# google/supersonic

Hardware: AMD Instinct MI355X
Metric: rows/sec filter->project->aggregate, 100M x 8 INT64/DOUBLE (higher is better)
Workload: dtype int64/f64; 1 GPU; Q-FPA-wide: SUM(a+b),COUNT(*),SUM(c),MIN(d),MAX(d0),SUM(d1),SUM(d2*d3) WHERE a>499 over a device-resident 100000000-row x 8-col block per GPU; rows_per_gpu=100000000, parallelism=single GPU, tile_rows=512, grid=768, lds_bytes=35568, specialized_stages=1

## Files before the change

include/ssgpu.h:

```cpp
#ifndef SSGPU_H_
#define SSGPU_H_

#include <stddef.h>
#include <stdint.h>

#ifdef __cplusplus
extern "C" {
#endif

#define SSGPU_ABI_VERSION 10

enum {
  SSGPU_INT32 = 1, SSGPU_INT64 = 2, SSGPU_UINT64 = 3, SSGPU_DATETIME = 4,
  SSGPU_DOUBLE = 5, SSGPU_BOOL = 6, SSGPU_UINT32 = 8, SSGPU_FLOAT = 9,
  SSGPU_DATE = 10, SSGPU_STRING = 0, SSGPU_BINARY = 7
};
enum { SSGPU_NOT_NULLABLE = 0, SSGPU_NULLABLE = 1 };
enum {
  SSGPU_SUM = 0, SSGPU_MIN = 1, SSGPU_MAX = 2, SSGPU_COUNT = 3,
  SSGPU_CONCAT = 4, SSGPU_FIRST = 5, SSGPU_LAST = 6,
  SSGPU_SUM_RESIDUAL = 100
};
enum { SSGPU_ASCENDING = 0, SSGPU_DESCENDING = 1 };
enum {
// ... 223 lines not shown
int64_t ssgpu_plan_memory_in_use(const ssgpu_plan* plan);

typedef struct ssgpu_stage_info {
  int32_t kind;
  int32_t group_shape;
  int32_t part_n;
  int32_t part_seg_growth;
  int32_t group_wgs_per_cu;
  int32_t reruns;
  int32_t sort_passes;
  int32_t sort_mode;
  int32_t specialized;
  int32_t plain_scatter;
  int32_t hot_keys;
  int32_t dense_slots;
  int32_t reserved[4];
} ssgpu_stage_info;
int32_t ssgpu_plan_stage_count(const ssgpu_plan* plan);
int ssgpu_plan_stage_info(const ssgpu_plan* plan, int32_t stage, ssgpu_stage_info* out);

int ssgpu_expr_bind(ssgpu_ctx* ctx, const ssgpu_attr* schema, int32_t n_attrs, const ssgpu_expr* exprs, int32_t n_exprs,
                    const int32_t* expr_args, int32_t n_expr_args, int32_t root, int64_t max_row_count, ssgpu_plan** out);
int64_t ssgpu_expr_row_capacity(const ssgpu_plan* bound);
int ssgpu_expr_evaluate(ssgpu_plan* bound, const ssgpu_column* cols, int32_t n_cols, int64_t rows, ssgpu_result** out);
int ssgpu_expr_evaluate_skip(ssgpu_plan* bound, const ssgpu_column* cols, int32_t n_cols, int64_t rows, uint8_t* const* skip, int32_t n_skip,
                             ssgpu_result** out);

int ssgpu_plan_set_option(ssgpu_plan* plan, const char* key, int64_t value);
int ssgpu_plan_run_best_effort(ssgpu_plan* plan, const ssgpu_column* cols, int32_t n_cols, int64_t rows, int64_t start_row,
                               int64_t* next_row, ssgpu_result** out);
int ssgpu_plan_run(ssgpu_plan* plan, const ssgpu_column* cols, int32_t n_cols,
// ... 74 lines not shown
```

supersonic_amd/_lib.py:

```python
import ctypes as C
import os

_HERE = os.path.dirname(os.path.abspath(__file__))
LIB_PATH = os.environ.get("SSGPU_LIB") or os.path.join(_HERE, "lib", "libssgpu.so")

INT32, INT64, UINT64, DATETIME, DOUBLE, BOOL, UINT32, FLOAT, DATE, STRING, BINARY = 1, 2, 3, 4, 5, 6, 8, 9, 10, 0, 7
NOT_NULLABLE, NULLABLE = 0, 1
SUM, MIN, MAX, COUNT, CONCAT, FIRST, LAST = 0, 1, 2, 3, 4, 5, 6
SUM_RESIDUAL = 100
ASCENDING, DESCENDING = 0, 1

OK = 0
ERROR_UNKNOWN = 100
ERROR_GENERAL_IO_ERROR = 101
ERROR_MEMORY_EXCEEDED = 102
ERROR_NOT_IMPLEMENTED = 103
ERROR_EVALUATION_ERROR = 104
ERROR_TOO_MANY_ROWS = 302
ERROR_ATTRIBUTE_COUNT_MISMATCH = 401
ERROR_ATTRIBUTE_TYPE_MISMATCH = 402
ERROR_ATTRIBUTE_MISSING = 403
ERROR_ATTRIBUTE_EXISTS = 404
ERROR_INVALID_ARGUMENT_TYPE = 405
ERROR_INVALID_ARGUMENT_VALUE = 407
# ... 37 lines not shown

class Op(C.Structure):
    _fields_ = [("kind", C.c_int32), ("child", C.c_int32), ("expr", C.c_int32), ("proj_first", C.c_int32),
                ("proj_n", C.c_int32), ("agg_first", C.c_int32), ("agg_n", C.c_int32), ("sort_first", C.c_int32),
                ("sort_n", C.c_int32), ("child2", C.c_int32), ("option0", C.c_int64),
                ("proj2_first", C.c_int32), ("proj2_n", C.c_int32), ("proj3_first", C.c_int32), ("proj3_n", C.c_int32)]


class MemoryStats(C.Structure):
    _fields_ = [(n, C.c_int64) for n in ("device_bytes", "pinned_bytes", "live_plans", "live_blocks", "events",
                                          "rtc_modules", "rtc_code_bytes", "rtc_compilations", "rtc_disk_hits")]


class StageInfo(C.Structure):
    _fields_ = [(n, C.c_int32) for n in ("kind", "group_shape", "part_n", "part_seg_growth", "group_wgs_per_cu", "reruns",
                                          "sort_passes", "sort_mode", "specialized", "plain_scatter", "hot_keys", "dense_slots")] + [("reserved", C.c_int32 * 4)]


class PlanDesc(C.Structure):
    _fields_ = [("input_schema", C.POINTER(Attr)), ("n_attrs", C.c_int32),
                ("ops", C.POINTER(Op)), ("n_ops", C.c_int32),
                ("exprs", C.POINTER(Expr)), ("n_exprs", C.c_int32),
                ("expr_args", C.POINTER(C.c_int32)), ("n_expr_args", C.c_int32),
                ("projs", C.POINTER(Proj)), ("n_projs", C.c_int32),
                ("aggs", C.POINTER(Agg)), ("n_aggs", C.c_int32),
                ("sortkeys", C.POINTER(SortKey)), ("n_sortkeys", C.c_int32),
                ("aux_schema", C.POINTER(Attr)), ("n_aux_attrs", C.c_int32)]


class Column(C.Structure):
    _fields_ = [("data", C.c_void_p), ("is_null", C.c_void_p)]
# ... 158 lines not shown
```

supersonic_amd/csrc/engine.h:

```cpp
#ifndef SSGPU_ENGINE_H_
#define SSGPU_ENGINE_H_

#include <stdint.h>
#include <map>
#include <memory>
#include <string>
#include <vector>

#include "../../include/ssgpu.h"
#include "vm.h"
#include "launch.h"

extern "C" int ssgpu_dict_create_sorted(const char* heap, const uint64_t* offsets, int64_t n, ssgpu_dict** out);

namespace ssgpu {

struct Status {
  int code = SSGPU_OK;
  std::string msg;
  bool ok() const { return code == SSGPU_OK; }
  static Status OK() { return Status(); }
  static Status Error(int c, const std::string& m) { Status s; s.code = c; s.msg = m; return s; }
};
#define SS_RETURN_IF_ERROR(expr) do { ::ssgpu::Status _s = (expr); if (!_s.ok()) return _s; } while (0)
// ... 69 lines not shown
  uint16_t op = 0;
  bool a_imm = false, b_imm = false;
  uint8_t imm_width = 8;
  bool dst_is_reg = true;
  int dst = -1;
  int a = -1, b = -1, c = -1, d = -1, e = -1;
  uint64_t imm = 0;
};
struct StagedInput { int col; bool is_null_mask; int reg; };

struct Program {
  std::vector<LInstr> code;
  std::vector<LReg> regs;
  std::vector<StagedInput> staged;
  std::vector<JoinGather> gathers;
  bool uses_math = false;
  uint32_t bytes_per_row = 0;
  uint32_t in_bytes_per_row = 0;
  int n_slots = 0;
  int n_outputs = 0;
  bool empty() const { return code.empty(); }
};

struct Stage {
  StageKind kind = STAGE_MATERIALIZE;
  Schema in_schema;
  Schema out_schema;
  Program main;
  Program count_pass;
  bool has_filter = false;
// ... 73 lines not shown
```

supersonic_amd/csrc/launch.h:

```cpp
#ifndef SSGPU_LAUNCH_H_
#define SSGPU_LAUNCH_H_

#ifndef __HIPCC_RTC__
#include <hip/hip_runtime_api.h>
#include <stdint.h>
#endif
#include "vm.h"

enum SlotKind {
  SLOT_SUM_INT = 0, SLOT_SUM_DD = 1, SLOT_MIN_U64 = 2, SLOT_MAX_U64 = 3, SLOT_MIN_F64 = 4,
  SLOT_MAX_F64 = 5, SLOT_FIRST = 6, SLOT_LAST = 7, SLOT_COUNT = 8
};
enum EmitKind {
  EMIT_U64 = 0, EMIT_I64KEY = 1, EMIT_U32 = 2, EMIT_I32KEY = 3, EMIT_F64 = 4, EMIT_F32 = 5,
  EMIT_DD_F64 = 6, EMIT_DD_F32 = 7, EMIT_U8 = 8,
  EMIT_DDRES_F64 = 9,
  EMIT_CNT_U64 = 20, EMIT_CNT_U32 = 21,
  EMIT_FKEY_F64 = 100, EMIT_FKEY_F32 = 101
};
#define SSGPU_STATE_ARRAYS 8

struct EmitDesc { void* data; uint8_t* is_null; int slot; int out_kind; };

struct GroupKeyOut { void* data; uint8_t* is_null; uint32_t shift, bits, nullbit, width; };
// ... 145 lines not shown
hipError_t ssgpu_launch_join_build(const JoinBuildParams& P, hipStream_t stream);
hipError_t ssgpu_launch_fill_u32(unsigned int* p, unsigned int v, size_t n, hipStream_t stream);
struct GroupInitParams {
  unsigned long long* keys; unsigned long long n_keys;
  unsigned long long* acc; const unsigned long long* pattern; unsigned int ng; unsigned long long n_acc;
  unsigned int* cnt; unsigned long long n_cnt;
  unsigned int* z[4]; unsigned long long nz[4];
  unsigned int n_rep, pad; unsigned long long rep_stride;
};
hipError_t ssgpu_launch_group_init(const GroupInitParams& P, hipStream_t stream);

hipError_t ssgpu_launch_pipeline(const VmParams& P, int K, int grid, hipStream_t stream);
#ifndef __HIPCC_RTC__
#include <string>
void* ssgpu_rtc_specialize(int device, const VmInstr* prog, int n_instr, int K, bool math, const uint32_t* staged_width, const uint32_t* staged_lds_off,
                           int n_staged, uint32_t static_lds, std::string* why);
hipError_t ssgpu_launch_pipeline_rtc(void* handle, const VmParams& P, int grid, bool static_lds, hipStream_t stream);
void* ssgpu_rtc_specialize_part_agg(int device, const unsigned long long* desc, int n_aggs, unsigned int rec_words, unsigned int n_gaggs, bool any_cnt,
                                    unsigned int lds_bytes, std::string* why, const PlainScatterParams* source = nullptr,
                                    bool dense = false,
                                    bool prefetch = false);
hipError_t ssgpu_launch_group_resident_rtc(void* handle, const PartAggParams& A, const PlainScatterParams& S, int grid, hipStream_t stream);
hipError_t ssgpu_launch_part_agg_rtc(void* handle, const PartAggParams& P, hipStream_t stream);
void* ssgpu_rtc_specialize_pscat(int device, const PlainScatterParams& S, const PscatGeom& g, std::string* why);
hipError_t ssgpu_launch_part_scatter_plain_rtc(void* handle, const PlainScatterParams& P, const PscatGeom& g, int grid, hipStream_t stream);
void* ssgpu_rtc_function(void* handle);
void ssgpu_rtc_release(void* handle);
void ssgpu_rtc_cached_only(bool on);
void ssgpu_rtc_mode(int mode);
int ssgpu_rtc_current_mode();
bool ssgpu_rtc_pending();
// ... 107 lines not shown
```

supersonic_amd/csrc/lower.cpp:

```cpp
#include "engine.h"

#include <algorithm>
#include <functional>
#include <sstream>
#include <string.h>

namespace ssgpu {

enum {
  OP_ADD = 0, OP_MULTIPLY = 4, OP_SUBTRACT = 8, OP_DIVIDE_QUIET = 13, OP_DIVIDE_NULLING = 14,
  OP_DIVIDE_SIGNALING = 15, OP_CPP_DIVIDE_NULLING = 18, OP_CPP_DIVIDE_SIGNALING = 19,
  OP_MODULUS_NULLING = 26, OP_MODULUS_SIGNALING = 27, OP_NEGATE = 36,
  OP_IS_ODD = 140, OP_IS_EVEN = 144, OP_IS_FINITE = 148, OP_IS_INF = 152, OP_IS_NAN = 156, OP_IS_NORMAL = 160,
  OP_ROUND_WITH_MULTIPLIER = 364, OP_EXP = 320, OP_LN_QUIET = 325, OP_LN_NULLING = 326, OP_LOG10_QUIET = 329, OP_LOG10_NULLING = 330, OP_POW_QUIET = 353,
  OP_POW_NULLING = 354, OP_POW_SIGNALING = 355, OP_LOG2_QUIET = 357, OP_LOG2_NULLING = 358, OP_SIN = 800, OP_COS = 804, OP_TAN = 808,
  OP_ASIN = 812, OP_ACOS = 816, OP_ATAN = 820, OP_ATAN2 = 824, OP_SINH = 828, OP_COSH = 832, OP_TANH = 836, OP_ASINH = 840,
  OP_ACOSH = 844, OP_ATANH = 848,
  OP_ROUND = 300, OP_TRUNC = 304, OP_CEIL_TO_INT = 308, OP_FLOOR_TO_INT = 312, OP_SQRT_QUIET = 333, OP_SQRT_NULLING = 334,
  OP_SQRT_SIGNALING = 335, OP_CEIL = 342, OP_FLOOR = 346, OP_ABS = 360, OP_AND = 40, OP_OR = 44,
  OP_AND_NOT = 48, OP_NOT = 52, OP_XOR = 56, OP_BITWISE_AND = 60, OP_BITWISE_OR = 64,
  OP_BITWISE_NOT = 68, OP_BITWISE_XOR = 72, OP_SHIFT_LEFT = 76, OP_SHIFT_RIGHT = 80,
  OP_BITWISE_ANDNOT = 84, OP_EQUAL = 100, OP_NOT_EQUAL = 104, OP_LESS = 116, OP_LESS_OR_EQUAL = 120,
  OP_IF = 204, OP_IF_NULL = 220, OP_IS_NULL = 224, OP_CAST_QUIET = 265
};
// ... 689 lines not shown
    if (fused_agg) {
      v.b = off(i.b);
      if (i.b_imm) v.d = pool;
    }
    v.imm = i.imm;
    if (i.op == VM_AND3 || i.op == VM_OR3) v.imm = (uint64_t)off(i.d) | ((uint64_t)off(i.e) << 32);
    out->push_back(v);
  }
  VmInstr nop; memset(&nop, 0, sizeof(nop)); nop.op = VM_NOP;
  nop.dst = nop.a = nop.b = nop.c = nop.d = VM_NONE;
  out->push_back(nop);
}

std::string disassemble(const Program& p) {
  std::ostringstream s;
  s << "  staged:";
  for (auto& st : p.staged) s << " r" << st.reg << "<-col" << st.col << (st.is_null_mask ? ".null" : "") << "(w" << p.regs[st.reg].width << ")";
  s << "\n  lds bytes/row: " << p.bytes_per_row << ", slots: " << p.n_slots << ", outputs: " << p.n_outputs << "\n";
  auto R = [&](int r) { return r < 0 ? std::string("-") : "r" + std::to_string(r) + "@" + std::to_string(p.regs[r].row_off); };
  for (size_t pc = 0; pc < p.code.size(); ++pc) {
    const LInstr& i = p.code[pc];
    s << "  " << pc << ": " << vm_op_name(i.op) << " dst=" << (i.dst_is_reg ? R(i.dst) : "#" + std::to_string(i.dst))
      << " a=" << (i.a_imm ? "imm" : R(i.a)) << " b=" << (i.b_imm ? "imm" : R(i.b)) << " c=" << R(i.c) << " d=" << R(i.d);
    if (i.e >= 0) s << " e=" << R(i.e);
    if (i.a_imm || i.b_imm || i.imm) s << " imm=0x" << std::hex << i.imm << std::dec;
    s << "\n";
  }
  return s.str();
}

// ... 210 lines not shown
    Val pv;
    SS_RETURN_IF_ERROR(em.value(pipe.filters[f], &pv));
    if (!pv.imm && pv.null < 0 && em.sel_by_depth.back() < 0) {
      em.sel_by_depth.push_back(pv.reg);
      continue;
    }
    int r = em.new_reg(1);
    LInstr& i = em.emit(VM_SEL_FROM_PRED);
    i.dst = r;
    if (pv.imm) { i.a_imm = true; i.imm = pv.bits; i.imm_width = 1; } else i.a = pv.reg;
    i.b = pv.null;
    i.c = em.sel_by_depth.back();
    em.sel_by_depth.push_back(r);
  }
  return Status::OK();
}

static int64_t staged_bytes(const Program& p) {
  int64_t b = 0;
  for (auto& s : p.staged) b += p.regs[s.reg].width;
  return b;
}

static bool has_sequential(const std::vector<AggPlan>& plans) { for (auto& ap : plans) if (ap.sequential) return true; return false; }
static Status take_sequential(std::vector<AggPlan>* plans, const Pipe& pipe, size_t first_out, std::vector<Stage::SeqSum>* out) {
  for (size_t j = 0; j < plans->size(); ++j) {
    AggPlan& ap = (*plans)[j];
    if (!ap.sequential) continue;
    const BExprP& src = pipe.cols[ap.input_pos].expr;
    if (src->kind != BExpr::INPUT) return Status::Error(SSGPU_ERROR_NOT_IMPLEMENTED, "SUM of a floating value into an integer output needs a stored input column");
// ... 88 lines not shown
        if (ap.distinct) { int nf; SS_RETURN_IF_ERROR(notfirst_for(ap, &nf)); nullreg = em.or_null(v.null, nf); }
        int order_reg = -1;
        if (ap.order_pos >= 0 && (ap.aggregation == SSGPU_FIRST || ap.aggregation == SSGPU_LAST)) {
          Val ov; SS_RETURN_IF_ERROR(em.value(pipe.cols[ap.order_pos].expr, &ov));
          order_reg = em.materialize(ov);
        }
        LInstr& i = em.emit(s.op); i.dst_is_reg = false; i.dst = (int)j; i.a = vr; i.b = nullreg; i.c = sel; i.d = order_reg;
      }
      ao.slot_kind = s.slot_kind; ao.emit_kind = s.emit_kind;
    }
    st->aggs.push_back(ao);
    Attr a; a.name = ap.out_name; a.dtype = ap.out_type; a.nullable = ap.result_nullable;
    st->out_schema.push_back(a);
  }
  st->main.n_slots = (int)plans.size();
  allocate_registers(&st->main);
  st->algorithmic_bytes_per_row = staged_bytes(st->main);
  st->has_filter = !pipe.filters.empty();
  return Status::OK();
}

static Status finish_scalar_agg(const PlanDesc& d, const ssgpu_op& op, const Pipe& pipe, Stage* st) {
  std::vector<AggPlan> plans;
  SS_RETURN_IF_ERROR(bind_aggregations(d, op.agg_first, op.agg_n, schema_of(pipe.cols), &plans));
  return finish_scalar_agg_bound(plans, pipe, st);
}

struct AggPlan;
static Status build_partition_programs(const struct Pipe& pipe, const std::vector<int>& kpos, const std::vector<AggPlan>& plans, Stage* st);

// ... 406 lines not shown
    if (st->has_filter) { i.b = rank; i.c = sel; }
  };
  for (size_t c = 0; c < pipe.cols.size(); ++c) {
    const BExprP& e = pipe.cols[c].expr;
    Val v; SS_RETURN_IF_ERROR(em.value(e, &v));
    store(v, v.width);
    if (e->nullable) {
      Val nv; nv.width = 1;
      if (v.null >= 0) nv.reg = v.null; else { nv.imm = true; nv.bits = 0; }
      store(nv, 1);
    }
    st->output_bytes_per_row += v.width + (e->nullable ? 1 : 0);
  }
  if (out_index > VM_MAX_OUTPUTS) return Status::Error(SSGPU_ERROR_NOT_IMPLEMENTED, "too many output columns for one pipeline");
  st->main.n_outputs = out_index;
  allocate_registers(&st->main);
  st->algorithmic_bytes_per_row = staged_bytes(st->main);
  return Status::OK();
}

static Pipe prune_to_used(const Pipe& pipe, std::vector<int>* kpos, std::vector<AggPlan>* plans) {
  std::vector<int> used;
  auto slot_of = [&](int pos) { for (size_t i = 0; i < used.size(); ++i) if (used[i] == pos) return (int)i; used.push_back(pos); return (int)used.size() - 1; };
  if (kpos) for (auto& k : *kpos) k = slot_of(k);
  for (auto& ap : *plans) if (ap.input_pos >= 0) ap.input_pos = slot_of(ap.input_pos);
  Pipe pruned = pipe; pruned.cols.clear();
  for (size_t i = 0; i < used.size(); ++i) { VCol c = pipe.cols[used[i]]; c.name = "c" + std::to_string(i); pruned.cols.push_back(c); }
  return pruned;
}
static int add_row_id_column(Pipe* pruned) {
// ... 633 lines not shown
```

supersonic_amd/csrc/pipeline_kernels.hip:

```cpp
#ifndef __HIPCC_RTC__
#include <hip/hip_runtime.h>
#include <stdint.h>
#endif
#include "vm.h"
#include "launch.h"
#ifdef SSGPU_RTC_NINSTR
#include "rtc_prog.h"
#endif

typedef unsigned long long u64;
typedef long long i64;
typedef unsigned int u32;
typedef int i32;
typedef unsigned char u8;

#ifdef SSGPU_PC_PROFILE
#define PC_PROF(...) __VA_ARGS__
#else
#define PC_PROF(...)
#endif
struct LdsBase {
  __device__ __forceinline__ char* operator+(u32 off) const {
    return (char*)(__attribute__((address_space(3))) char*)off;
  }
// ... 151 lines not shown
  return 0xFFFFFFFFu;
}

typedef u32 u32x4 __attribute__((ext_vector_type(4)));
typedef u32 u32x2 __attribute__((ext_vector_type(2)));

#if defined(SSGPU_RTC_NINSTR) && !defined(SSGPU_RTC_DYNAMIC_STAGING)
#define STAGED_WIDTH(P, s) kRtcStagedWidth[s]
#define STAGED_LDS_OFF(P, s) kRtcStagedOff[s]
#define STAGED_COUNT(P) SSGPU_RTC_NSTAGED
#else
#define STAGED_WIDTH(P, s) (P).staged[s].width
#define STAGED_LDS_OFF(P, s) (P).staged[s].lds_off
#define STAGED_COUNT(P) (P).n_staged
#endif
template <int K>
__device__ __forceinline__ void load_unit(const VmParams& P, int u, i64 tile_base, int t, u32x4& v) {
  const int s = u / K, k = u % K;
  const char* const src0 = reinterpret_cast<const char*>(P.staged[s].src);
  const u32 w = STAGED_WIDTH(P, s);
  if (src0 == nullptr) return;
  const u32 p = (u32)(k * VM_COMPUTE_THREADS + t);
  if (w == 8) {
    v = __builtin_nontemporal_load(reinterpret_cast<const u32x4*>(src0 + (tile_base << 3) + (size_t)(p * 16u)));
  } else if (w == 4) {
    const u32x2 x = __builtin_nontemporal_load(reinterpret_cast<const u32x2*>(src0 + (tile_base << 2) + (size_t)(p * 8u)));
    v[0] = x[0]; v[1] = x[1];
  } else if ((reinterpret_cast<uintptr_t>(src0) & 1) == 0) {
    v[0] = (u32)__builtin_nontemporal_load(reinterpret_cast<const unsigned short*>(src0 + tile_base + (size_t)(p * 2u)));
  } else {
// ... 2 lines not shown
  }
}

template <int K>
__device__ __forceinline__ void commit_unit(const VmParams& P, int u, u32x4 v, int t) {
  const int s = u / K, k = u % K;
  const u32 w = STAGED_WIDTH(P, s);
  const u32 p = (u32)(k * VM_COMPUTE_THREADS + t);
  char* const dst = smem + STAGED_LDS_OFF(P, s);
  if (w == 8) *reinterpret_cast<u32x4*>(dst + p * 16u) = v;
  else if (w == 4) { u32x2 x = {v[0], v[1]}; *reinterpret_cast<u32x2*>(dst + p * 8u) = x; }
  else *reinterpret_cast<unsigned short*>(dst + p * 2u) = (unsigned short)v[0];
}

template <int K>
__device__ __forceinline__ void stage_units_direct(const VmParams& P, int u_begin, int u_end, i64 tile_base, u32 tile_valid, int t) {
  for (int u = u_begin; u < u_end; ++u) {
    const int s = u / K, k = u % K;
    const char* const src0 = reinterpret_cast<const char*>(P.staged[s].src);
    const u32 w = STAGED_WIDTH(P, s);
    const u32 p = (u32)(k * VM_COMPUTE_THREADS + t), r0 = 2u * p;
    char* const dst = smem + STAGED_LDS_OFF(P, s);
    const bool v0 = src0 != nullptr && r0 < tile_valid, v1 = src0 != nullptr && r0 + 1u < tile_valid;
    if (w == 8) {
      const u64* src = reinterpret_cast<const u64*>(src0) + tile_base + r0;
      u64 a = v0 ? src[0] : 0ull, b = v1 ? src[1] : 0ull;
      reinterpret_cast<u64*>(dst)[r0] = a; reinterpret_cast<u64*>(dst)[r0 + 1u] = b;
    } else if (w == 4) {
      const u32* src = reinterpret_cast<const u32*>(src0) + tile_base + r0;
      u32 a = v0 ? src[0] : 0u, b = v1 ? src[1] : 0u;
      reinterpret_cast<u32*>(dst)[r0] = a; reinterpret_cast<u32*>(dst)[r0 + 1u] = b;
    } else {
      const u8* src = reinterpret_cast<const u8*>(src0) + tile_base + r0;
      u8 a = v0 ? src[0] : (u8)0, b = v1 ? src[1] : (u8)0;
      reinterpret_cast<u8*>(dst)[r0] = a; reinterpret_cast<u8*>(dst)[r0 + 1u] = b;
    }
  }
}
// ... 337 lines not shown
  PC_PROF(if (P.debug_pc) for (int i = t; i <= P.n_instr; i += VM_COMPUTE_THREADS) reinterpret_cast<u64*>(smem + P.debug_pc_lds_off)[i] = 0ull;)
  __syncthreads();

  u32x4 pf[VM_PF_UNITS];
#pragma unroll
  for (int u = 0; u < VM_PF_UNITS; ++u) pf[u] = u32x4{0u, 0u, 0u, 0u};
  const int n_pf = n_units < VM_PF_UNITS ? n_units : VM_PF_UNITS;
  {
    const i64 tb = (i64)vm_first_tile * tile_rows;
    if (n_my_tiles > 0 && tb + tile_rows <= vm_n_rows) {
#pragma unroll
      for (int u = 0; u < VM_PF_UNITS; ++u)
        if (u < n_pf) load_unit<K>(P, u, tb, t, pf[u]);
    }
  }

  u64 dbg_wait = 0;
  const u64 dbg_t0 = P.debug ? __builtin_amdgcn_s_memtime() : 0;
  const ProgPtr prog = prog0;
  for (int it = 0; it < n_my_tiles; ++it) {
    const int tile = vm_first_tile + it * (int)gridDim.x;
    const i64 tile_base = (i64)tile * tile_rows;
    const u32 tile_valid = (u32)((vm_n_rows - tile_base) < (i64)tile_rows ? (vm_n_rows - tile_base) : (i64)tile_rows);
    const u64 tw0 = (P.debug || P.debug_pc) ? __builtin_amdgcn_s_memtime() : 0;
    __builtin_amdgcn_s_setprio(VM_STAGE_PRIO);
    if (tile_valid == (u32)tile_rows) {
      int tc = t;
      asm volatile("" : "+v"(tc));
#pragma unroll
      for (int u = 0; u < VM_PF_UNITS; ++u)
        if (u < n_pf) commit_unit<K>(P, u, pf[u], tc);
      if (P.debug) dbg_wait += __builtin_amdgcn_s_memtime() - tw0;
      if (n_units > VM_PF_UNITS) stage_units_direct<K>(P, VM_PF_UNITS, n_units, tile_base, tile_valid, t);
    } else {
      stage_units_direct<K>(P, 0, n_units, tile_base, tile_valid, t);
    }
    {
      const i64 tb = tile_base + (i64)gridDim.x * tile_rows;
      if (it + 1 < n_my_tiles && tb + tile_rows <= vm_n_rows) {
        int tl = t;
        asm volatile("" : "+v"(tl));
#pragma unroll
        for (int u = 0; u < VM_PF_UNITS; ++u)
          if (u < n_pf) load_unit<K>(P, u, tb, tl, pf[u]);
      }
    }

    __builtin_amdgcn_s_setprio(0);
#ifdef SSGPU_RTC_NINSTR
#define VM_PC_LOOP _Pragma("unroll") for (int pc = 0; pc < SSGPU_RTC_NINSTR; ++pc)
#define VM_FETCH_NEXT(pc) u32x8{kRtcProg[pc][0], kRtcProg[pc][1], kRtcProg[pc][2], kRtcProg[pc][3], kRtcProg[pc][4], kRtcProg[pc][5], kRtcProg[pc][6], kRtcProg[pc][7]}
    (void)prog;
    u32x8 raw_next = VM_FETCH_NEXT(0);
#else
#define VM_PC_LOOP for (int pc = 0; pc < P.n_instr; ++pc)
#define VM_FETCH_NEXT(pc) prog[pc]
    u32x8 raw_next = prog[0];
#endif
    PC_PROF(u64 dbg_pc_last = 0;
    if (P.debug_pc) { dbg_pc_last = __builtin_amdgcn_s_memtime(); if (t == 0) reinterpret_cast<u64*>(smem + P.debug_pc_lds_off)[P.n_instr] += dbg_pc_last - tw0; })
#ifdef SSGPU_RTC_NINSTR
#include "rtc_steps.h"
#else
    VM_PC_LOOP {
#include "vm_body.inc"
    }
#endif
    PC_PROF(if (P.debug_pc && P.n_instr > 0 && t == 0) reinterpret_cast<u64*>(smem + P.debug_pc_lds_off)[P.n_instr - 1] += __builtin_amdgcn_s_memtime() - dbg_pc_last;)
  }

  if (vm_nan_seen && P.error_flag) atomicOr(P.error_flag, SSGPU_FLAG_NAN_IN_MINMAX);
  if (P.part_n && P.tile_counts) {
    __syncthreads();
    const u32* h = reinterpret_cast<const u32*>(smem + P.part_lds_off);
    for (u32 i = (u32)t; i < P.part_n; i += VM_COMPUTE_THREADS) P.tile_counts[(u64)i * gridDim.x + blockIdx.x] = h[i] < P.part_seg_cap ? h[i] : P.part_seg_cap;
  }
  if (P.group.local_capacity) {
    const VmGroupTable& G = P.group;
    __syncthreads();
    const u32 ng = G.n_gaggs;
    u32 occupied = 0;
    for (u32 e = (u32)t; e < G.local_capacity; e += VM_COMPUTE_THREADS) {
      const u64 key = reinterpret_cast<const u64*>(smem + G.local_keys_off)[e];
// ... 1283 lines not shown
```

supersonic_amd/csrc/rtc.cpp:

```cpp
#include <dirent.h>
#include <dlfcn.h>
#include <fcntl.h>
#include <errno.h>
#include <sys/stat.h>
#include <sys/types.h>
#include <unistd.h>
#include <hip/hip_runtime_api.h>
#include <stdint.h>
#include <stdio.h>
#include <stdlib.h>
#include <string.h>

#include <algorithm>
#include <atomic>
#include <condition_variable>
#include <deque>
#include <map>
#include <mutex>
#include <string>
#include <thread>
#include <vector>

#include "launch.h"
#include "vm.h"
// ... 360 lines not shown
}
void ssgpu_rtc_trim(int keep) {
  std::vector<Entry*> victims;
  { std::lock_guard<std::mutex> lock(g_mutex); trim_idle_locked(keep < 0 ? 0 : (size_t)keep, &victims); }
  unload_entries(victims);
}

void ssgpu_rtc_stats(long long* modules, long long* code_bytes, long long* compilations, long long* disk_hits) {
  if (modules) *modules = g_modules.load();
  if (code_bytes) *code_bytes = g_code_bytes.load();
  if (compilations) *compilations = g_compilations.load();
  if (disk_hits) *disk_hits = g_disk_hits.load();
}

void* ssgpu_rtc_specialize(int device, const VmInstr* prog, int n_instr, int K, bool math, const uint32_t* staged_width, const uint32_t* staged_lds_off,
                           int n_staged, uint32_t static_lds, std::string* why) {
  if (n_instr <= 0 || n_instr > 96) { *why = "program length outside the specialised range"; return nullptr; }
  if (tls_mode == 0 && !rtc().ok) { *why = "libhiprtc is not available"; return nullptr; }
  std::string key = "pipeline|" + std::string(reinterpret_cast<const char*>(prog), (size_t)(n_instr + 1) * sizeof(VmInstr));
  key += "|" + std::to_string(device) + "|" + std::to_string(K) + (math ? "m" : "n") + "|" + std::to_string(static_lds);
  for (int i = 0; i < n_staged; ++i) key += "|" + std::to_string(staged_width[i]) + "@" + std::to_string(staged_lds_off[i]);
  if (const char* env = getenv("SSGPU_RTC_FLAGS")) key += std::string("|") + env;
  return acquire(key, why, [&]() -> Job {
    static_assert(sizeof(VmInstr) == 32, "the specialised kernel reads instructions as 8 dwords");
    std::string table = "static constexpr unsigned int kRtcProg[" + std::to_string(n_instr + 1) + "][8] = {";
    const uint32_t* w = reinterpret_cast<const uint32_t*>(prog);
    for (int i = 0; i <= n_instr; ++i) {
      table += i ? ",{" : "{";
      for (int j = 0; j < 8; ++j) { table += std::to_string(w[i * 8 + j]) + (j < 7 ? "u," : "u"); }
      table += "}";
    }
    table += "};\n";
    table += "#define SSGPU_RTC_NSTAGED " + std::to_string(n_staged) + "\n";
    std::string sw = "static constexpr unsigned int kRtcStagedWidth[" + std::to_string(n_staged + 1) + "] = {", so = "static constexpr unsigned int kRtcStagedOff[" + std::to_string(n_staged + 1) + "] = {";
    for (int i = 0; i < n_staged; ++i) { sw += std::to_string(staged_width[i]) + "u,"; so += std::to_string(staged_lds_off[i]) + "u,"; }
    table += sw + "0u};\n" + so + "0u};\n";
    std::string steps;
    for (int i = 0; i < n_instr; ++i) steps += "    { constexpr int pc = " + std::to_string(i) + ";\n#include \"vm_body.inc\"\n    }\n";
    std::vector<std::string> defines = {"-DSSGPU_RTC_NINSTR=" + std::to_string(n_instr)};
    if (static_lds) defines.push_back("-DSSGPU_RTC_STATIC_LDS=" + std::to_string((static_lds + 15u) & ~15u));
    const std::string expr = "ssgpu_pipeline_kernel<" + std::to_string(K) + ", " + (math ? "true" : "false") + ">";
    Job job; job.prog_name = "ssgpu_pipeline_rtc.hip"; job.gen_headers = {{"rtc_prog.h", table}, {"rtc_steps.h", steps}}; job.device = device; job.defines = defines; job.expr = expr;
    return job;
  });
}

void* ssgpu_rtc_specialize_part_agg(int device, const unsigned long long* desc, int n_aggs, unsigned int rec_words, unsigned int n_gaggs, bool any_cnt,
                                    unsigned int lds_bytes, std::string* why, const PlainScatterParams* source, bool dense, bool prefetch) {
  if (n_aggs <= 0 || n_aggs > VM_MAX_AGG_SLOTS) { *why = "aggregate count outside the specialised range"; return nullptr; }
  if (tls_mode == 0 && !rtc().ok) { *why = "libhiprtc is not available"; return nullptr; }
  const int maxw = rec_words <= 8 ? 8 : rec_words <= 16 ? 16 : SSGPU_PART_MAX_WORDS;
// ... 87 lines not shown
```

supersonic_amd/csrc/runtime.cpp:

```cpp
#include <hip/hip_runtime_api.h>

#include <atomic>
#include <map>
#include <mutex>
#include <stdio.h>
#include <string.h>
#include <algorithm>
#include <cmath>
#include <string>
#include <unistd.h>
#include <thread>
#include <unordered_set>
#include <vector>
#include <deque>
#include <functional>

#include "engine.h"

using namespace ssgpu;

#define HIP_TRY(ctx, expr)                                                          \
  do {                                                                               \
    hipError_t _e = (expr);                                                          \
    if (_e != hipSuccess) {                                                          \
// ... 949 lines not shown

int upload_program(ssgpu_ctx* c, const Program& prog, const ProgramLayout& L, DevBuf* dev, int* n_instr, std::vector<VmInstr>* scratch) {
  finalize_program(prog, L, scratch);
  *n_instr = (int)prog.code.size();
  HIP_TRY(c, dev->ensure(std::max<size_t>(1, scratch->size()) * sizeof(VmInstr)));
  if (!scratch->empty())
    HIP_TRY(c, hipMemcpyAsync(dev->p, scratch->data(), scratch->size() * sizeof(VmInstr), hipMemcpyHostToDevice, c->stream));
  HIP_TRY(c, hipStreamSynchronize(c->stream));
  return SSGPU_OK;
}

static void staged_table(const Program& prog, const ProgramLayout& L, std::vector<uint32_t>* width, std::vector<uint32_t>* off) {
  width->clear(); off->clear();
  for (auto& sgd : prog.staged) { width->push_back(prog.regs[sgd.reg].width); off->push_back(prog.regs[sgd.reg].row_off * (uint32_t)(VM_TILE_UNIT * L.K)); }
}
void* rtc_for(ssgpu_plan* p, StageExec& ex, StageExec::RtcSlot& slot, const Program& prog, const ProgramLayout& L, const std::vector<VmInstr>& host_prog,
              int n_instr, uint32_t lds_bytes, const char* what) {
  if (!p->specialize) return nullptr;
  ssgpu_ctx* c = p->ctx;
  const uint32_t need_static = lds_bytes > 64u * 1024u ? ((lds_bytes + 15u) & ~15u) : 0u;
  if (slot.tried && slot.static_lds == need_static && !slot.ask_again() && !slot.stronger_mode_now()) return slot.h;
  if (slot.h) { (void)hipStreamSynchronize(c->stream); slot.drop(); }
  const bool was_pending = slot.pending;
  slot.tried = true; slot.static_lds = need_static;
  std::vector<uint32_t> sw, so; staged_table(prog, L, &sw, &so);
  std::string why;
  slot.h = ssgpu_rtc_specialize(c->device, host_prog.data(), n_instr, L.K, prog.uses_math, sw.data(), so.data(), (int)sw.size(), need_static, &why);
  slot.asked();
  if (!slot.h && ex.rtc_why.empty()) ex.rtc_why = std::string(what) + why;
  if (slot.h && was_pending) ex.rtc_why.clear();
  return slot.h;
}

int prepare_stage(ssgpu_plan* p, size_t si) {
  ssgpu_ctx* c = p->ctx;
  Stage& st = p->stages[si];
  StageExec& ex = p->exec[si];
  if (st.main.empty()) return SSGPU_OK;
  ProgramLayout L = layout_program(st.main, c->opt);
  if (ex.prog_main.p && L.K == ex.lay.K) return SSGPU_OK;
  ex.lay = L;
  int rc = upload_program(c, st.main, L, &ex.prog_main, &ex.n_instr_main, &p->host_prog_scratch);
// ... 171 lines not shown
  P->n_rows_dev = in.rows_dev;
  P->row_id_base = row_id_base;
  P->tile_rows = VM_TILE_UNIT * L.K;
  P->n_tiles = (int)((in.rows + P->tile_rows - 1) / P->tile_rows);
  P->acc_lds_off = L.acc_off;
  P->scratch_lds_off = L.scratch_off;
  P->imm_pool_lds_off = L.imm_pool_off;
  P->const_lds_off = L.imm_pool_off + 16u * (uint32_t)prog.code.size();
  P->lds_bytes = L.lds_bytes;
  for (size_t i = 0; i < prog.staged.size(); ++i) {
    const StagedInput& s = prog.staged[i];
    P->staged[i].src = s.is_null_mask ? (const void*)in.cols[s.col].is_null : in.cols[s.col].data;
    P->staged[i].lds_off = prog.regs[s.reg].row_off * (uint32_t)P->tile_rows;
    P->staged[i].width = prog.regs[s.reg].width;
  }
}

int ensure_out_cols(ssgpu_ctx* c, const Stage& st, StageExec& ex, int64_t rows) {
  ex.out.resize(st.out_schema.size());
  size_t total = 0;
  for (size_t i = 0; i < st.out_schema.size(); ++i) {
    OutCol& oc = ex.out[i];
    oc.width = (uint32_t)dtype_width(st.out_schema[i].dtype);
    oc.nullable = st.out_schema[i].nullable;
    total += (size_t)std::max<int64_t>(rows, 1) * (oc.width + (oc.nullable ? 1u : 0u));
  }
  if (c->out_arena && total >= kBlockArenaMin && st.out_schema.size() > 1) {
    auto pitch = [](size_t bytes) { return ((bytes + (2u << 20) - 1) / (2u << 20)) * (2u << 20) + kBlockColumnSkew; };
    bool fits = ex.out_arena.p != nullptr;
    for (size_t i = 0; i < ex.out.size() && fits; ++i)
// ... 1733 lines not shown
  return SSGPU_OK;
}
int32_t ssgpu_plan_stage_count(const ssgpu_plan* p) { return p ? (int32_t)p->stages.size() : 0; }
int ssgpu_plan_stage_info(const ssgpu_plan* p, int32_t stage, ssgpu_stage_info* out) {
  if (!p || !out || stage < 0 || stage >= (int32_t)p->stages.size()) return SSGPU_ERROR_INVALID_ARGUMENT_VALUE;
  const StageExec& ex = p->exec[stage];
  memset(out, 0, sizeof(*out));
  out->kind = (int32_t)p->stages[stage].kind;
  out->group_shape = ex.last_group_shape; out->part_n = (int32_t)ex.part_n; out->part_seg_growth = (int32_t)ex.part_seg_growth;
  out->group_wgs_per_cu = ex.group_wgs; out->reruns = ex.last_reruns;
  out->sort_passes = ex.last_sort_passes; out->sort_mode = ex.last_sort_mode;
  out->specialized = (ex.rtc_main.h ? 1 : 0) + (ex.rtc_pscatter.h ? 2 : 0) + (ex.rtc_part.h ? 4 : 0) + (ex.rtc_plain.h ? 8 : 0) + (ex.rtc_resident.h ? 16 : 0);
  out->plain_scatter = ex.last_plain_scatter ? 1 : 0;
  out->hot_keys = (int32_t)ex.hot_n;
  out->dense_slots = ex.dense.on ? (int32_t)ex.dense.slots : 0;
  return SSGPU_OK;
}
void ssgpu_specialized_kernels_trim(int32_t keep) { ssgpu_rtc_trim(keep); }
int ssgpu_memory_stats(ssgpu_memory_stats_t* out) {
  if (!out) return SSGPU_ERROR_INVALID_ARGUMENT_VALUE;
  memset(out, 0, sizeof(*out));
  out->device_bytes = g_dev_bytes.load(); out->pinned_bytes = g_pinned_bytes.load();
  out->live_plans = g_live_plans.load(); out->live_blocks = g_live_blocks.load(); out->events = g_events.load();
  long long m = 0, b = 0, n = 0, d = 0;
  ssgpu_rtc_stats(&m, &b, &n, &d);
  out->rtc_modules = m; out->rtc_code_bytes = b; out->rtc_compilations = n; out->rtc_disk_hits = d;
  return SSGPU_OK;
}
int ssgpu_plan_set_memory_limit(ssgpu_plan* p, int64_t bytes) {
  if (!p) return SSGPU_ERROR_INVALID_ARGUMENT_VALUE;
// ... 1216 lines not shown
```

supersonic_amd/csrc/vm.h:

```cpp
#ifndef SSGPU_VM_H_
#define SSGPU_VM_H_

#ifdef __HIPCC_RTC__
typedef signed char int8_t; typedef unsigned char uint8_t; typedef short int16_t; typedef unsigned short uint16_t;
typedef int int32_t; typedef unsigned int uint32_t; typedef long int64_t; typedef unsigned long uint64_t; typedef unsigned long uintptr_t;
typedef int hipError_t; typedef struct ihipStream_t* hipStream_t;
#else
#include <stdint.h>
#endif

#define VM_NONE 0xFFFFFFFFu
enum { VM_MATH_EXP = 1, VM_MATH_LN, VM_MATH_LOG10, VM_MATH_LOG2, VM_MATH_SIN, VM_MATH_COS, VM_MATH_TAN, VM_MATH_ASIN, VM_MATH_ACOS,
       VM_MATH_ATAN, VM_MATH_SINH, VM_MATH_COSH, VM_MATH_TANH, VM_MATH_ASINH, VM_MATH_ACOSH, VM_MATH_ATANH, VM_MATH_POW, VM_MATH_ATAN2 };
#ifndef VM_THREADS
#define VM_THREADS 256
#endif
#ifndef VM_PF_UNITS
#define VM_PF_UNITS 8
#endif
#ifndef VM_WAVES_PER_EU
#define VM_WAVES_PER_EU 4
#endif
#ifndef VM_STAGE_PRIO
#define VM_STAGE_PRIO 1
// ... 159 lines not shown
#define VM_MERGE_ADD_F64_HI 4u
#define VM_SLOT_LOCAL 0x80000000u
#define VM_KEY_EMPTY 0xFFFFFFFFFFFFFFFFull

struct VmJoin {
  const unsigned long long* keys;
  const unsigned int* rows;
  const unsigned int* special;
  uint32_t capacity_mask;
  uint32_t answer_slot;
  const unsigned long long* keys_hi;
};
struct VmJoinCol { const void* data; const unsigned char* is_null; };
#define VM_MAX_JOINS 2
#define VM_MAX_JOIN_COLS 24

struct VmParams {
  const VmInstr* prog;
  int32_t n_instr;
  int32_t n_staged;
  int32_t n_outputs;
  int32_t n_slots;
  int64_t n_rows;
  int64_t row_id_base;
  int32_t tile_rows;
  int32_t n_tiles;
  uint32_t acc_lds_off;
  uint32_t scratch_lds_off;
  uint32_t imm_pool_lds_off;
  uint32_t const_lds_off;
// ... 4 lines not shown
  uint64_t slot_init1[VM_FAST_SLOTS];
  int32_t slot_kind[VM_FAST_SLOTS];
  VmAccRec* wg_partials;
  unsigned int* tile_counts;
  uint32_t part_n;
  uint32_t part_lds_off;
  uint32_t part_seg_cap;
  unsigned int* part_overflow;
  const unsigned int* tile_offsets;
  const unsigned long long* n_rows_dev;
  unsigned int* error_flag;
  unsigned long long* debug;
  unsigned long long* debug_pc;
  uint32_t debug_pc_lds_off;
  uint32_t uses_math;
  VmGroupTable group;
  VmJoin join[VM_MAX_JOINS];
  VmJoinCol join_cols[VM_MAX_JOIN_COLS];
  VmStagedCol staged[VM_MAX_STAGED];
  VmOutCol outputs[VM_MAX_OUTPUTS];
};
static_assert(sizeof(VmParams) <= 4096, "VmParams must fit the 4 KiB kernel-argument block");

#define VM_FLAG_XCD_CHUNKS 1u

#ifndef __HIPCC__
static inline const char* vm_op_name(uint16_t op) {
  static const char* names[] = {
#define X(n) #n,
      VM_OPS(X)
// ... 10 lines not shown
```

Before: 101.9 billion rows/s.

## Evaluate simple filter predicates early and skip loading columns for rejected rows

Extracts simple column-vs-constant comparison terms from the filter's AND chain and moves the predicate columns to the front of the staged list. The kernel loads those columns one tile ahead, computes per-row keep bits, and loads the remaining columns only for rows that pass, also masking the direct-staging path. The goal is to cut global-memory reads of non-predicate columns when the filter rejects rows. The cost is a deeper prefetch pipeline with more registers and a dependency between the predicate loads and the other loads. With row-level masking inside cache lines, the reduction in DRAM traffic may be small unless whole lines are rejected.

After: 100.8 billion rows/s. -1.1%, worse.

```diff
diff --git a/include/ssgpu.h b/include/ssgpu.h
--- a/include/ssgpu.h
+++ b/include/ssgpu.h
@@ -261,7 +261,8 @@
   int32_t plain_scatter;
   int32_t hot_keys;
   int32_t dense_slots;
-  int32_t reserved[4];
+  int32_t pred_first;
+  int32_t reserved[3];
 } ssgpu_stage_info;
 int32_t ssgpu_plan_stage_count(const ssgpu_plan* plan);
 int ssgpu_plan_stage_info(const ssgpu_plan* plan, int32_t stage, ssgpu_stage_info* out);
diff --git a/supersonic_amd/_lib.py b/supersonic_amd/_lib.py
--- a/supersonic_amd/_lib.py
+++ b/supersonic_amd/_lib.py
@@ -75,7 +75,7 @@
 
 class StageInfo(C.Structure):
     _fields_ = [(n, C.c_int32) for n in ("kind", "group_shape", "part_n", "part_seg_growth", "group_wgs_per_cu", "reruns",
-                                          "sort_passes", "sort_mode", "specialized", "plain_scatter", "hot_keys", "dense_slots")] + [("reserved", C.c_int32 * 4)]
+                                          "sort_passes", "sort_mode", "specialized", "plain_scatter", "hot_keys", "dense_slots", "pred_first")] + [("reserved", C.c_int32 * 3)]
 
 
 class PlanDesc(C.Structure):
diff --git a/supersonic_amd/csrc/engine.h b/supersonic_amd/csrc/engine.h
--- a/supersonic_amd/csrc/engine.h
+++ b/supersonic_amd/csrc/engine.h
@@ -107,6 +107,8 @@
   std::vector<LReg> regs;
   std::vector<StagedInput> staged;
   std::vector<JoinGather> gathers;
+  std::vector<VmPredTerm> pred;
+  int pred_cols = 0;
   bool uses_math = false;
   uint32_t bytes_per_row = 0;
   uint32_t in_bytes_per_row = 0;
diff --git a/supersonic_amd/csrc/launch.h b/supersonic_amd/csrc/launch.h
--- a/supersonic_amd/csrc/launch.h
+++ b/supersonic_amd/csrc/launch.h
@@ -183,7 +183,7 @@
 #ifndef __HIPCC_RTC__
 #include <string>
 void* ssgpu_rtc_specialize(int device, const VmInstr* prog, int n_instr, int K, bool math, const uint32_t* staged_width, const uint32_t* staged_lds_off,
-                           int n_staged, uint32_t static_lds, std::string* why);
+                           int n_staged, uint32_t static_lds, std::string* why, const VmPred* pred = nullptr);
 hipError_t ssgpu_launch_pipeline_rtc(void* handle, const VmParams& P, int grid, bool static_lds, hipStream_t stream);
 void* ssgpu_rtc_specialize_part_agg(int device, const unsigned long long* desc, int n_aggs, unsigned int rec_words, unsigned int n_gaggs, bool any_cnt,
                                     unsigned int lds_bytes, std::string* why, const PlainScatterParams* source = nullptr,
diff --git a/supersonic_amd/csrc/lower.cpp b/supersonic_amd/csrc/lower.cpp
--- a/supersonic_amd/csrc/lower.cpp
+++ b/supersonic_amd/csrc/lower.cpp
@@ -727,6 +727,7 @@
 
 std::string disassemble(const Program& p) {
   std::ostringstream s;
+  if (!p.pred.empty()) s << "  predicate-first: " << p.pred.size() << " term(s) over the first " << p.pred_cols << " staged column(s)\n";
   s << "  staged:";
   for (auto& st : p.staged) s << " r" << st.reg << "<-col" << st.col << (st.is_null_mask ? ".null" : "") << "(w" << p.regs[st.reg].width << ")";
   s << "\n  lds bytes/row: " << p.bytes_per_row << ", slots: " << p.n_slots << ", outputs: " << p.n_outputs << "\n";
@@ -967,6 +968,56 @@
     em.sel_by_depth.push_back(r);
   }
   return Status::OK();
+}
+
+static void and_chain(const BExprP& e, std::vector<BExprP>* out) {
+  if (e->kind == BExpr::OP && e->op == OP_AND && e->args.size() == 2) { and_chain(e->args[0], out); and_chain(e->args[1], out); }
+  else out->push_back(e);
+}
+static void find_early_predicate(Emitter& em, const Pipe& pipe, int sel, Program* p) {
+  p->pred.clear(); p->pred_cols = 0;
+  if (pipe.filters.empty() || !pipe.joins.empty() || sel < 0) return;
+  for (auto& f : pipe.filters) if (em.may_fail(f)) return;
+  for (auto& c : pipe.cols) if (em.may_fail(c.expr)) return;
+  for (auto& i : p->code) {
+    const bool agg = i.op >= VM_AGG_COUNT && i.op <= VM_AGG_SUM_F64_MUL;
+    const bool storec = i.op == VM_STOREC_8 || i.op == VM_STOREC_32 || i.op == VM_STOREC_64 || i.op == VM_STORE_ROWID;
+    if (agg || storec) { if (i.dst_is_reg || i.c != sel) return; continue; }
+    if (i.op == VM_SEL_RANK) { if (i.a != sel) return; continue; }
+    if (!i.dst_is_reg || i.op >= VM_SEL_COUNT) return;
+  }
+  std::vector<BExprP> terms;
+  for (auto& f : pipe.filters) and_chain(f, &terms);
+  std::vector<int> cols;
+  for (auto& e : terms) {
+    if ((int)p->pred.size() >= VM_MAX_PRED) break;
+    if (e->kind != BExpr::OP || e->args.size() != 2 || !(e->op == OP_LESS || e->op == OP_LESS_OR_EQUAL || e->op == OP_EQUAL || e->op == OP_NOT_EQUAL)) continue;
+    const bool col_left = e->args[0]->kind == BExpr::INPUT && e->args[1]->kind == BExpr::CONST;
+    const bool col_right = e->args[1]->kind == BExpr::INPUT && e->args[0]->kind == BExpr::CONST;
+    if (!col_left && !col_right) continue;
+    const BExprP& ce = e->args[col_left ? 0 : 1]; const BExprP& ke = e->args[col_left ? 1 : 0];
+    const MT m = mtype(ce->dtype);
+    if (ce->nullable || m != mtype(ke->dtype) || !(m == M_I32 || m == M_U32 || m == M_I64 || m == M_U64 || m == M_F32 || m == M_F64)) continue;
+    size_t ci = std::find(cols.begin(), cols.end(), ce->input_col) - cols.begin();
+    if (ci == cols.size()) {
+      if ((int)cols.size() >= VM_PQ_UNITS) continue;
+      cols.push_back(ce->input_col);
+    }
+    VmPredTerm t; memset(&t, 0, sizeof(t));
+    t.col = (uint16_t)ci;
+    t.op = (uint8_t)((e->op == OP_LESS ? VM_PC_LT : e->op == OP_LESS_OR_EQUAL ? VM_PC_LE : e->op == OP_EQUAL ? VM_PC_EQ : VM_PC_NE) | (col_left ? VM_PC_COL_LEFT : 0));
+    t.kind = (uint8_t)(m == M_I32 ? VM_PK_I32 : m == M_U32 ? VM_PK_U32 : m == M_I64 ? VM_PK_I64 : m == M_U64 ? VM_PK_U64 : m == M_F32 ? VM_PK_F32 : VM_PK_F64);
+    t.imm = mwidth(m) == 4 ? (ke->bits & 0xFFFFFFFFull) : ke->bits;
+    p->pred.push_back(t);
+  }
+  if (p->pred.empty()) return;
+  std::vector<StagedInput> front, rest;
+  for (int col : cols)
+    for (auto& s : p->staged) if (s.col == col && !s.is_null_mask) front.push_back(s);
+  if (front.size() != cols.size()) { p->pred.clear(); return; }
+  for (auto& s : p->staged) if (s.is_null_mask || std::find(cols.begin(), cols.end(), s.col) == cols.end()) rest.push_back(s);
+  p->staged = front; p->staged.insert(p->staged.end(), rest.begin(), rest.end());
+  p->pred_cols = (int)cols.size();
 }
 
 static int64_t staged_bytes(const Program& p) {
@@ -1085,6 +1136,7 @@
     st->out_schema.push_back(a);
   }
   st->main.n_slots = (int)plans.size();
+  find_early_predicate(em, pipe, sel, &st->main);
   allocate_registers(&st->main);
   st->algorithmic_bytes_per_row = staged_bytes(st->main);
   st->has_filter = !pipe.filters.empty();
@@ -1521,6 +1573,7 @@
   }
   if (out_index > VM_MAX_OUTPUTS) return Status::Error(SSGPU_ERROR_NOT_IMPLEMENTED, "too many output columns for one pipeline");
   st->main.n_outputs = out_index;
+  if (st->has_filter) find_early_predicate(em, pipe, sel, &st->main);
   allocate_registers(&st->main);
   st->algorithmic_bytes_per_row = staged_bytes(st->main);
   return Status::OK();
diff --git a/supersonic_amd/csrc/pipeline_kernels.hip b/supersonic_amd/csrc/pipeline_kernels.hip
--- a/supersonic_amd/csrc/pipeline_kernels.hip
+++ b/supersonic_amd/csrc/pipeline_kernels.hip
@@ -189,6 +189,62 @@
 #define STAGED_LDS_OFF(P, s) (P).staged[s].lds_off
 #define STAGED_COUNT(P) (P).n_staged
 #endif
+#if defined(SSGPU_RTC_NINSTR) && !defined(SSGPU_RTC_DYNAMIC_STAGING)
+#define PRED_TERMS(P) SSGPU_RTC_NPRED
+#define PRED_COLS(P) SSGPU_RTC_NPRED_COLS
+#define PRED_COL(P, j) kRtcPred[j][0]
+#define PRED_OP(P, j) kRtcPred[j][1]
+#define PRED_KIND(P, j) kRtcPred[j][2]
+#define PRED_IMM(P, j) (((u64)kRtcPred[j][4] << 32) | (u64)kRtcPred[j][3])
+#else
+#define PRED_TERMS(P) (int)(P).pred.n_terms
+#define PRED_COLS(P) (int)(P).pred.n_cols
+#define PRED_COL(P, j) (u32)(P).pred.term[j].col
+#define PRED_OP(P, j) (u32)(P).pred.term[j].op
+#define PRED_KIND(P, j) (u32)(P).pred.term[j].kind
+#define PRED_IMM(P, j) (u64)(P).pred.term[j].imm
+#endif
+__device__ __forceinline__ bool pred_term_row(u32 kind, u32 op, u64 imm, u64 x) {
+  bool lt, gt, eq;
+  switch (kind) {
+    case VM_PK_I32: { const i32 a = (i32)(u32)x, b = (i32)(u32)imm; lt = a < b; gt = a > b; eq = a == b; } break;
+    case VM_PK_U32: { const u32 a = (u32)x, b = (u32)imm; lt = a < b; gt = a > b; eq = a == b; } break;
+    case VM_PK_I64: { const i64 a = (i64)x, b = (i64)imm; lt = a < b; gt = a > b; eq = a == b; } break;
+    case VM_PK_U64: { const u64 a = x, b = imm; lt = a < b; gt = a > b; eq = a == b; } break;
+    case VM_PK_F32: { const float a = __uint_as_float((u32)x), b = __uint_as_float((u32)imm); lt = a < b; gt = a > b; eq = a == b; } break;
+    default: { const double a = u2d(x), b = u2d(imm); lt = a < b; gt = a > b; eq = a == b; } break;
+  }
+  const bool left = (op & VM_PC_COL_LEFT) != 0;
+  switch (op & 3u) {
+    case VM_PC_LT: return left ? lt : gt;
+    case VM_PC_LE: return left ? (lt || eq) : (gt || eq);
+    case VM_PC_EQ: return eq;
+    default: return !eq;
+  }
+}
+template <int K>
+__device__ __forceinline__ u32 pred_keep_bits(const VmParams& P, const u32x4 (&pq)[VM_PQ_UNITS]) {
+  u32 keep = ~0u;
+#pragma unroll
+  for (int j = 0; j < VM_MAX_PRED; ++j) {
+    if (j < PRED_TERMS(P)) {
+      const u32 col = PRED_COL(P, j), op = PRED_OP(P, j), kind = PRED_KIND(P, j);
+      const u64 imm = PRED_IMM(P, j);
+      const bool wide = kind == VM_PK_I64 || kind == VM_PK_U64 || kind == VM_PK_F64;
+#pragma unroll
+      for (int k = 0; k < K && k < VM_PQ_UNITS; ++k) {
+        const u32 u = col * (u32)K + (u32)k;
+        const u32x4 v = u == 0u ? pq[0] : pq[VM_PQ_UNITS - 1];
+        const u64 x0 = wide ? (((u64)v[1] << 32) | v[0]) : (u64)v[0];
+        const u64 x1 = wide ? (((u64)v[3] << 32) | v[2]) : (u64)v[1];
+        const u32 fail = (pred_term_row(kind, op, imm, x0) ? 0u : 1u) | (pred_term_row(kind, op, imm, x1) ? 0u : 2u);
+        keep &= ~(fail << (2 * k));
+      }
+    }
+  }
+  return keep;
+}
+
 template <int K>
 __device__ __forceinline__ void load_unit(const VmParams& P, int u, i64 tile_base, int t, u32x4& v) {
   const int s = u / K, k = u % K;
@@ -221,14 +277,14 @@
 }
 
 template <int K>
-__device__ __forceinline__ void stage_units_direct(const VmParams& P, int u_begin, int u_end, i64 tile_base, u32 tile_valid, int t) {
+__device__ __forceinline__ void stage_units_direct(const VmParams& P, int u_begin, int u_end, i64 tile_base, u32 tile_valid, int t, u32 keep = ~0u) {
   for (int u = u_begin; u < u_end; ++u) {
     const int s = u / K, k = u % K;
     const char* const src0 = reinterpret_cast<const char*>(P.staged[s].src);
     const u32 w = STAGED_WIDTH(P, s);
     const u32 p = (u32)(k * VM_COMPUTE_THREADS + t), r0 = 2u * p;
     char* const dst = smem + STAGED_LDS_OFF(P, s);
-    const bool v0 = src0 != nullptr && r0 < tile_valid, v1 = src0 != nullptr && r0 + 1u < tile_valid;
+    const bool v0 = src0 != nullptr && r0 < tile_valid && ((keep >> (2 * k)) & 1u), v1 = src0 != nullptr && r0 + 1u < tile_valid && ((keep >> (2 * k + 1)) & 1u);
     if (w == 8) {
       const u64* src = reinterpret_cast<const u64*>(src0) + tile_base + r0;
       u64 a = v0 ? src[0] : 0ull, b = v1 ? src[1] : 0ull;
@@ -596,6 +652,19 @@
         if (u < n_pf) load_unit<K>(P, u, tb, t, pf[u]);
     }
   }
+  const int n_pq = (K <= VM_PQ_UNITS && PRED_TERMS(P) > 0) ? PRED_COLS(P) * K : 0;
+  u32x4 pq[VM_PQ_UNITS];
+#pragma unroll
+  for (int u = 0; u < VM_PQ_UNITS; ++u) pq[u] = u32x4{0u, 0u, 0u, 0u};
+  u32 keep_cur = ~0u, keep_next = ~0u;
+  if (n_pq > 0) {
+    const i64 tb = ((i64)vm_first_tile + (i64)gridDim.x) * tile_rows;
+    if (n_my_tiles > 1 && tb + tile_rows <= vm_n_rows) {
+#pragma unroll
+      for (int u = 0; u < VM_PQ_UNITS; ++u)
+        if (u < n_pq) load_unit<K>(P, u, tb, t, pq[u]);
+    }
+  }
 
   u64 dbg_wait = 0;
   const u64 dbg_t0 = P.debug ? __builtin_amdgcn_s_memtime() : 0;
@@ -613,7 +682,7 @@
       for (int u = 0; u < VM_PF_UNITS; ++u)
         if (u < n_pf) commit_unit<K>(P, u, pf[u], tc);
       if (P.debug) dbg_wait += __builtin_amdgcn_s_memtime() - tw0;
-      if (n_units > VM_PF_UNITS) stage_units_direct<K>(P, VM_PF_UNITS, n_units, tile_base, tile_valid, t);
+      if (n_units > VM_PF_UNITS) stage_units_direct<K>(P, VM_PF_UNITS, n_units, tile_base, tile_valid, t, keep_cur);
     } else {
       stage_units_direct<K>(P, 0, n_units, tile_base, tile_valid, t);
     }
@@ -622,9 +691,30 @@
       if (it + 1 < n_my_tiles && tb + tile_rows <= vm_n_rows) {
         int tl = t;
         asm volatile("" : "+v"(tl));
-#pragma unroll
-        for (int u = 0; u < VM_PF_UNITS; ++u)
-          if (u < n_pf) load_unit<K>(P, u, tb, tl, pf[u]);
+        if (n_pq > 0) {
+          keep_next = pred_keep_bits<K>(P, pq);
+#pragma unroll
+          for (int u = 0; u < VM_PQ_UNITS; ++u)
+            if (u < n_pq) pf[u] = pq[u];
+#pragma unroll
+          for (int u = 0; u < VM_PF_UNITS; ++u)
+            if (u >= n_pq && u < n_pf) {
+              pf[u] = u32x4{0u, 0u, 0u, 0u};
+              if ((keep_next >> (2 * (u % K))) & 3u) load_unit<K>(P, u, tb, tl, pf[u]);
+            }
+          const i64 tb2 = tb + (i64)gridDim.x * tile_rows;
+          if (it + 2 < n_my_tiles && tb2 + tile_rows <= vm_n_rows) {
+#pragma unroll
+            for (int u = 0; u < VM_PQ_UNITS; ++u)
+              if (u < n_pq) load_unit<K>(P, u, tb2, tl, pq[u]);
+          }
+        } else {
+#pragma unroll
+          for (int u = 0; u < VM_PF_UNITS; ++u)
+            if (u < n_pf) load_unit<K>(P, u, tb, tl, pf[u]);
+        }
+      } else {
+        keep_next = ~0u;
       }
     }
 
@@ -649,6 +739,7 @@
     }
 #endif
     PC_PROF(if (P.debug_pc && P.n_instr > 0 && t == 0) reinterpret_cast<u64*>(smem + P.debug_pc_lds_off)[P.n_instr - 1] += __builtin_amdgcn_s_memtime() - dbg_pc_last;)
+    keep_cur = keep_next;
   }
 
   if (vm_nan_seen && P.error_flag) atomicOr(P.error_flag, SSGPU_FLAG_NAN_IN_MINMAX);
diff --git a/supersonic_amd/csrc/rtc.cpp b/supersonic_amd/csrc/rtc.cpp
--- a/supersonic_amd/csrc/rtc.cpp
+++ b/supersonic_amd/csrc/rtc.cpp
@@ -398,12 +398,17 @@
 }
 
 void* ssgpu_rtc_specialize(int device, const VmInstr* prog, int n_instr, int K, bool math, const uint32_t* staged_width, const uint32_t* staged_lds_off,
-                           int n_staged, uint32_t static_lds, std::string* why) {
+                           int n_staged, uint32_t static_lds, std::string* why, const VmPred* pred) {
   if (n_instr <= 0 || n_instr > 96) { *why = "program length outside the specialised range"; return nullptr; }
   if (tls_mode == 0 && !rtc().ok) { *why = "libhiprtc is not available"; return nullptr; }
   std::string key = "pipeline|" + std::string(reinterpret_cast<const char*>(prog), (size_t)(n_instr + 1) * sizeof(VmInstr));
   key += "|" + std::to_string(device) + "|" + std::to_string(K) + (math ? "m" : "n") + "|" + std::to_string(static_lds);
   for (int i = 0; i < n_staged; ++i) key += "|" + std::to_string(staged_width[i]) + "@" + std::to_string(staged_lds_off[i]);
+  VmPred q; memset(&q, 0, sizeof(q));
+  if (pred && pred->n_terms) q = *pred;
+  key += "|q" + std::to_string(q.n_terms) + "/" + std::to_string(q.n_cols);
+  for (uint32_t i = 0; i < q.n_terms; ++i)
+    key += "|" + std::to_string(q.term[i].col) + "," + std::to_string(q.term[i].op) + "," + std::to_string(q.term[i].kind) + "," + std::to_string((unsigned long long)q.term[i].imm);
   if (const char* env = getenv("SSGPU_RTC_FLAGS")) key += std::string("|") + env;
   return acquire(key, why, [&]() -> Job {
     static_assert(sizeof(VmInstr) == 32, "the specialised kernel reads instructions as 8 dwords");
@@ -419,6 +424,12 @@
     std::string sw = "static constexpr unsigned int kRtcStagedWidth[" + std::to_string(n_staged + 1) + "] = {", so = "static constexpr unsigned int kRtcStagedOff[" + std::to_string(n_staged + 1) + "] = {";
     for (int i = 0; i < n_staged; ++i) { sw += std::to_string(staged_width[i]) + "u,"; so += std::to_string(staged_lds_off[i]) + "u,"; }
     table += sw + "0u};\n" + so + "0u};\n";
+    table += "#define SSGPU_RTC_NPRED " + std::to_string(q.n_terms) + "\n#define SSGPU_RTC_NPRED_COLS " + std::to_string(q.n_cols) + "\n";
+    table += "static constexpr unsigned int kRtcPred[" + std::to_string(VM_MAX_PRED) + "][5] = {";
+    for (int i = 0; i < VM_MAX_PRED; ++i)
+      table += std::string(i ? ",{" : "{") + std::to_string(q.term[i].col) + "u," + std::to_string(q.term[i].op) + "u," + std::to_string(q.term[i].kind) + "u," +
+               std::to_string((uint32_t)q.term[i].imm) + "u," + std::to_string((uint32_t)(q.term[i].imm >> 32)) + "u}";
+    table += "};\n";
     std::string steps;
     for (int i = 0; i < n_instr; ++i) steps += "    { constexpr int pc = " + std::to_string(i) + ";\n#include \"vm_body.inc\"\n    }\n";
     std::vector<std::string> defines = {"-DSSGPU_RTC_NINSTR=" + std::to_string(n_instr)};
diff --git a/supersonic_amd/csrc/runtime.cpp b/supersonic_amd/csrc/runtime.cpp
--- a/supersonic_amd/csrc/runtime.cpp
+++ b/supersonic_amd/csrc/runtime.cpp
@@ -987,6 +987,12 @@
   width->clear(); off->clear();
   for (auto& sgd : prog.staged) { width->push_back(prog.regs[sgd.reg].width); off->push_back(prog.regs[sgd.reg].row_off * (uint32_t)(VM_TILE_UNIT * L.K)); }
 }
+static void pred_table(const Program& prog, int K, VmPred* out) {
+  memset(out, 0, sizeof(*out));
+  if (prog.pred.empty() || prog.pred_cols * K > VM_PQ_UNITS) return;
+  out->n_terms = (uint32_t)prog.pred.size(); out->n_cols = (uint32_t)prog.pred_cols;
+  for (size_t i = 0; i < prog.pred.size() && i < VM_MAX_PRED; ++i) out->term[i] = prog.pred[i];
+}
 void* rtc_for(ssgpu_plan* p, StageExec& ex, StageExec::RtcSlot& slot, const Program& prog, const ProgramLayout& L, const std::vector<VmInstr>& host_prog,
               int n_instr, uint32_t lds_bytes, const char* what) {
   if (!p->specialize) return nullptr;
@@ -998,7 +1004,8 @@
   slot.tried = true; slot.static_lds = need_static;
   std::vector<uint32_t> sw, so; staged_table(prog, L, &sw, &so);
   std::string why;
-  slot.h = ssgpu_rtc_specialize(c->device, host_prog.data(), n_instr, L.K, prog.uses_math, sw.data(), so.data(), (int)sw.size(), need_static, &why);
+  VmPred pred; pred_table(prog, L.K, &pred);
+  slot.h = ssgpu_rtc_specialize(c->device, host_prog.data(), n_instr, L.K, prog.uses_math, sw.data(), so.data(), (int)sw.size(), need_static, &why, &pred);
   slot.asked();
   if (!slot.h && ex.rtc_why.empty()) ex.rtc_why = std::string(what) + why;
   if (slot.h && was_pending) ex.rtc_why.clear();
@@ -1200,6 +1207,7 @@
     P->staged[i].lds_off = prog.regs[s.reg].row_off * (uint32_t)P->tile_rows;
     P->staged[i].width = prog.regs[s.reg].width;
   }
+  pred_table(prog, L.K, &P->pred);
 }
 
 int ensure_out_cols(ssgpu_ctx* c, const Stage& st, StageExec& ex, int64_t rows) {
@@ -2963,6 +2971,7 @@
   out->plain_scatter = ex.last_plain_scatter ? 1 : 0;
   out->hot_keys = (int32_t)ex.hot_n;
   out->dense_slots = ex.dense.on ? (int32_t)ex.dense.slots : 0;
+  if (ex.prog_main.p) { VmPred pred; pred_table(p->stages[stage].main, ex.lay.K, &pred); out->pred_first = (int32_t)pred.n_terms; }
   return SSGPU_OK;
 }
 void ssgpu_specialized_kernels_trim(int32_t keep) { ssgpu_rtc_trim(keep); }
diff --git a/supersonic_amd/csrc/vm.h b/supersonic_amd/csrc/vm.h
--- a/supersonic_amd/csrc/vm.h
+++ b/supersonic_amd/csrc/vm.h
@@ -197,6 +197,23 @@
 struct VmJoinCol { const void* data; const unsigned char* is_null; };
 #define VM_MAX_JOINS 2
 #define VM_MAX_JOIN_COLS 24
+
+#define VM_MAX_PRED 4
+#define VM_PQ_UNITS 2
+enum { VM_PK_I32 = 0, VM_PK_U32, VM_PK_I64, VM_PK_U64, VM_PK_F32, VM_PK_F64 };
+enum { VM_PC_LT = 0, VM_PC_LE, VM_PC_EQ, VM_PC_NE, VM_PC_COL_LEFT = 4 };
+struct VmPredTerm {
+  uint16_t col;
+  uint8_t op;
+  uint8_t kind;
+  uint32_t pad;
+  uint64_t imm;
+};
+struct VmPred {
+  uint32_t n_terms;
+  uint32_t n_cols;
+  VmPredTerm term[VM_MAX_PRED];
+};
 
 struct VmParams {
   const VmInstr* prog;
@@ -231,6 +248,7 @@
   unsigned long long* debug_pc;
   uint32_t debug_pc_lds_off;
   uint32_t uses_math;
+  VmPred pred;
   VmGroupTable group;
   VmJoin join[VM_MAX_JOINS];
   VmJoinCol join_cols[VM_MAX_JOIN_COLS];
```
